# HumanCompatibleAI/overcooked_ai

Hardware: NVIDIA H100
Metric: env-steps/sec (joint transitions) (higher is better)
Workload: dtype int32

## Files before the change

### overcooked_ai_b200/csrc/ovc_b200.cu

```cuda
#include <cuda.h>
#include <cuda_runtime.h>
#include <stdint.h>
#include <stdio.h>
#include <stdlib.h>
#include <string.h>

#include "../../include/ovc_b200.h"
#include "ovc_step.cuh"

namespace ovc {

static thread_local char g_err[512] = "";

static int fail(int code, const char *msg) {
    snprintf(g_err, sizeof g_err, "%s", msg);
    return code;
}
static int fail(int code, const char *msg, long long value) {
    snprintf(g_err, sizeof g_err, "%s (got %lld)", msg, value);
    return code;
}
static int cuda_fail(cudaError_t e, const char *what) {
    snprintf(g_err, sizeof g_err, "%s: %s", what, cudaGetErrorString(e));
    return OVC_E_CUDA;
// ... 225 lines not shown
        else bulk_load_1d(tile, a.state + env0 * S, live_bytes, bar);
    }
    int2 act = make_int2(OVC_A_STAY, OVC_A_STAY);
    if (live) act = load_action<WIDE>(a, env);
    __syncthreads();
    mbar_wait(bar, 0);
    asm volatile("griddepcontrol.launch_dependents;" ::: "memory");

    if (live) {
        SmemRec<S, IO == 1 ? C::SWZ : 0> r{tile, (uint32_t)threadIdx.x * S * 4};
        auto run = [&](auto tb) {
            for (int t = 0; t < T; t++) {
                const long long idx = (long long)t * a.n_envs + env;
                int2 nxt = act;
                if (t + 1 < T) nxt = load_action<WIDE>(a, idx + a.n_envs);
                StepOut o;
                step_core<RS>(r, tb, a.start_records, S, act.x, act.y, a.horizon, a.flags, RS ? &a.rs : nullptr, env, a.n_layouts, o);
                write_outputs<WIDE>(a, idx, o);
                act = nxt;
            }
        };
        if (n_tbl) run(TblS{tbl});
        else run(TblG{reinterpret_cast<const char *>(a.layouts)});
    }
    fence_async_smem();
    __syncthreads();
    if (threadIdx.x == 0) {
        if (IO == 1) tma_store_2d(&tmap, 0, (int)(env0 * C::ROWS_PER_ENV), tile);
        else bulk_store_1d(a.state + env0 * S, tile, live_bytes);
        bulk_commit();
        bulk_wait_read<0>();
    }
}

}

#include "ovc_rollout.cuh"

namespace ovc {

__global__ void reset_kernel(const int32_t *__restrict__ start_records, int n_layouts, int32_t *__restrict__ state,
                             const int32_t *__restrict__ env_layout, const int32_t *__restrict__ mask,
                             long long n_envs, int S) {
    const int cpr = S / 4;
    const long long i = (long long)blockIdx.x * blockDim.x + threadIdx.x;
    if (i >= n_envs * cpr) return;
    const long long env = i / cpr;
    const int c = (int)(i % cpr);
    if (mask && mask[env] == 0) return;
    int lid = env_layout ? env_layout[env] : (state[env * S + 3] & 0xFF);
    if (lid < 0 || lid >= n_layouts) lid = 0;
    reinterpret_cast<int4 *>(state)[i] = __ldg(reinterpret_cast<const int4 *>(start_records) + (long long)lid * cpr + c);
}

__global__ void reset_random_kernel(const ovc_layout_t *__restrict__ layouts, int n_layouts,
                                    const int32_t *__restrict__ start_records, int32_t *__restrict__ state,
                                    const int32_t *__restrict__ env_layout, const int32_t *__restrict__ mask,
                                    long long n_envs, int S, const ovc_random_start_t rs) {
    const long long env = (long long)blockIdx.x * blockDim.x + threadIdx.x;
    if (env >= n_envs) return;
    if (mask && mask[env] == 0) return;
    int32_t *rec = state + env * S;
    const unsigned old = (unsigned)rec[3];
    int lid = env_layout ? env_layout[env] : (int)(old & 0xFF);
    const unsigned episode = ((old >> 16) + 1u) & 0xFFFFu;
    if (rs.random_layout) lid = random_layout_id(rs, (uint64_t)env, episode, n_layouts);
    if (lid < 0 || lid >= n_layouts) lid = 0;
    const ovc_layout_t *L = layouts + lid;
    random_start_record([&](int w, int32_t v) { rec[w] = v; }, S, start_records + (size_t)lid * S, L->cook_time, L->free_pos,
                        L->n_free, L->n_pots, lid, rs, (uint64_t)env, episode);
}

typedef CUresult (*encode_tiled_fn)(CUtensorMap *, CUtensorMapDataType, cuuint32_t, void *, const cuuint64_t *,
                                    const cuuint64_t *, const cuuint32_t *, const cuuint32_t *, CUtensorMapInterleave,
                                    CUtensorMapSwizzle, CUtensorMapL2promotion, CUtensorMapFloatOOBfill);

static encode_tiled_fn get_encode_fn() {
    static encode_tiled_fn fn = nullptr;
    static bool tried = false;
    if (!tried) {
        tried = true;
        void *p = nullptr;
        cudaDriverEntryPointQueryResult q;
        if (cudaGetDriverEntryPoint("cuTensorMapEncodeTiled", &p, cudaEnableDefault, &q) == cudaSuccess &&
            q == cudaDriverEntryPointSuccess)
            fn = (encode_tiled_fn)p;
    }
    return fn;
}

template <int S>
static int make_tmap(CUtensorMap *m, int32_t *state, long long n_envs, int box_rows = Cfg<S>::BOX_ROWS) {
    using C = Cfg<S>;
    encode_tiled_fn enc = get_encode_fn();
    if (!enc) return fail(OVC_E_CUDA, "cuTensorMapEncodeTiled entry point not available");
    cuuint64_t dims[2] = {(cuuint64_t)C::ROW_WORDS, (cuuint64_t)(n_envs * C::ROWS_PER_ENV)};
    cuuint64_t strides[1] = {(cuuint64_t)C::ROW_WORDS * 4};
    cuuint32_t box[2] = {(cuuint32_t)C::ROW_WORDS, (cuuint32_t)box_rows};
    cuuint32_t estr[2] = {1, 1};
    CUresult r = enc(m, CU_TENSOR_MAP_DATA_TYPE_INT32, 2, state, dims, strides, box, estr, CU_TENSOR_MAP_INTERLEAVE_NONE,
                     S == 16 ? CU_TENSOR_MAP_SWIZZLE_64B : CU_TENSOR_MAP_SWIZZLE_128B, CU_TENSOR_MAP_L2_PROMOTION_NONE,
                     CU_TENSOR_MAP_FLOAT_OOB_FILL_NONE);
    if (r != CUDA_SUCCESS) return fail(OVC_E_CUDA, "cuTensorMapEncodeTiled failed", (long long)r);
    return OVC_OK;
}

struct OutFmt {
    int act, sparse, shaped, done, events;
    bool stream;
    bool missing(const void *act_p, const void *sparse_p, const void *shaped_p, const void *done_p, const void *events_p) const {
        return !act_p || !events_p || (sparse && !sparse_p) || (shaped && !shaped_p) || (done && !stream && !done_p);
    }
    bool wide() const { return act == 8 && sparse == 4; }
};

static OutFmt formats_of(int flags) {
    OutFmt f;
    f.act = (flags & OVC_F_ACT_PACKED) ? 1 : (flags & OVC_F_ACT_U8) ? 2 : 8;
    f.stream = flags & OVC_F_OUT_STREAM;
    if (f.stream) f.sparse = 2, f.shaped = 0, f.done = 2, f.events = 4;
    else if (flags & OVC_F_OUT_CODES) f.sparse = 0, f.shaped = 0, f.done = 0, f.events = 2;
    else if (flags & OVC_F_OUT_PACKED) f.sparse = 2, f.shaped = 2, f.done = 0, f.events = 2;
    else if (flags & OVC_F_OUT_NARROW) f.sparse = 2, f.shaped = 2, f.done = 1, f.events = 8;
    else f.sparse = 4, f.shaped = 8, f.done = 4, f.events = 8;
    return f;
}

template <int S, int IO>
static cudaError_t launch_one(const CUtensorMap &tmap, const StepArgs &a, unsigned grid, size_t smem, cudaStream_t st) {
    using C = Cfg<S>;
    cudaLaunchConfig_t cfg;
    memset(&cfg, 0, sizeof cfg);
    cfg.gridDim = dim3(grid), cfg.blockDim = dim3(C::TILE), cfg.dynamicSmemBytes = smem, cfg.stream = st;
    cudaLaunchAttribute attr[1];
    attr[0].id = cudaLaunchAttributeProgrammaticStreamSerialization;
    attr[0].val.programmaticStreamSerializationAllowed = 1;
    cfg.attrs = attr;
    cfg.numAttrs = (a.flags & OVC_F_PDL) ? 1 : 0;
    const bool wide = formats_of(a.flags).wide();
    if (a.has_rs)
        return wide ? cudaLaunchKernelEx(&cfg, step_kernel<S, IO, true, true>, tmap, a)
                    : cudaLaunchKernelEx(&cfg, step_kernel<S, IO, true, false>, tmap, a);
    return wide ? cudaLaunchKernelEx(&cfg, step_kernel<S, IO, false, true>, tmap, a)
                : cudaLaunchKernelEx(&cfg, step_kernel<S, IO, false, false>, tmap, a);
}

template <int S, int TILE>
static int launch_rollout(const StepArgs &a, cudaStream_t st) {
    using C = RollCfg<S, TILE>;
    CUtensorMap tmap;
    memset(&tmap, 0, sizeof tmap);
    int rc = make_tmap<S>(&tmap, a.state, a.n_envs, C::BOX_ROWS);
    if (rc) return rc;
    const size_t smem = C::smem_bytes(a.n_layouts);
    const OutFmt f = formats_of(a.flags);
    const bool wide = f.wide(), stream = f.stream;
    void (*kern)(const CUtensorMap, const StepArgs) =
        a.has_rs ? (wide ? rollout_kernel<S, TILE, true, FMT_WIDE> : stream ? rollout_kernel<S, TILE, true, FMT_STREAM> : rollout_kernel<S, TILE, true, FMT_HOST>)
                 : (wide ? rollout_kernel<S, TILE, false, FMT_WIDE> : stream ? rollout_kernel<S, TILE, false, FMT_STREAM> : rollout_kernel<S, TILE, false, FMT_HOST>);
    if (smem > 48 * 1024) {
        cudaError_t e = cudaFuncSetAttribute(kern, cudaFuncAttributeMaxDynamicSharedMemorySize, (int)smem);
        if (e != cudaSuccess) return cuda_fail(e, "rollout kernel shared-memory attribute");
    }
    const long long grid = (a.n_envs + TILE - 1) / TILE;
    StepArgs ka = a;
    ka.flags &= ~F_K5_NO_PREFETCH;
#if OVC_K5_PREFETCH > 1
    {
        int dev = 0, n_sm = 0, per_sm = 0;
        cudaError_t e = cudaGetDevice(&dev);
        if (e == cudaSuccess) e = cudaDeviceGetAttribute(&n_sm, cudaDevAttrMultiProcessorCount, dev);
        if (e == cudaSuccess) e = cudaOccupancyMaxActiveBlocksPerMultiprocessor(&per_sm, kern, TILE, smem);
        if (e != cudaSuccess) return cuda_fail(e, "rollout kernel occupancy");
        const long long warps = grid * (TILE / 32);
        if (grid <= (long long)per_sm * n_sm && (warps >= 24LL * n_sm || warps < 12LL * n_sm)) ka.flags |= F_K5_NO_PREFETCH;
    }
#endif
    cudaLaunchConfig_t cfg;
    memset(&cfg, 0, sizeof cfg);
    cfg.gridDim = dim3((unsigned)grid), cfg.blockDim = dim3(TILE), cfg.dynamicSmemBytes = smem, cfg.stream = st;
    cudaLaunchAttribute attr[1];
    attr[0].id = cudaLaunchAttributeProgrammaticStreamSerialization;
    attr[0].val.programmaticStreamSerializationAllowed = 1;
    cfg.attrs = attr;
    cfg.numAttrs = 0;
    cudaError_t e = cudaLaunchKernelEx(&cfg, kern, tmap, ka);
    if (e != cudaSuccess) return cuda_fail(e, "rollout kernel launch");
    return OVC_OK;
}

static int rollout_tile(int S, long long n_envs, int n_layouts) {
    static int forced = -1;
    if (forced < 0) {
        const char *e = getenv("OVC_K5_TILE");
        forced = e ? atoi(e) : 0;
    }
    (void)n_envs;
    if (S > 32) return 64;
    if (forced == 32 || forced == 64 || forced == 128) return forced;
    return n_layouts >= 3 ? 128 : 64;
}

static bool use_rollout_kernel(const StepArgs &a, int io) {
    static int off = -1;
    if (off < 0) {
        const char *e = getenv("OVC_K5_LEGACY");
        off = e && atoi(e) ? 1 : 0;
    }
    const bool stream = a.flags & OVC_F_OUT_STREAM;
    return (!off || stream) && (a.n_steps > 1 || stream) && a.n_steps <= ROLLOUT_MAX_STEPS && io == 1 && a.n_layouts <= MAX_SMEM_LAYOUTS;
}

template <int S>
static int launch_rollout_tiled(const StepArgs &a, cudaStream_t st) {
    if constexpr (S > 32) {
        return launch_rollout<S, 64>(a, st);
    } else {
        switch (rollout_tile(S, a.n_envs, a.n_layouts)) {
        case 32: return launch_rollout<S, 32>(a, st);
        case 64: return launch_rollout<S, 64>(a, st);
        default: return launch_rollout<S, 128>(a, st);
        }
    }
}

template <int S>
static int launch_rollout_any(const StepArgs &a0, cudaStream_t st) {
    long long max_steps = 0xFFFFFFFFLL / a0.n_envs - 1;
    {
        static long long cap = -1;
        if (cap < 0) {
            const char *e = getenv("OVC_K5_MAX_LAUNCH_STEPS");
            cap = e ? atoll(e) : 0;
        }
        if (cap > 0 && cap < max_steps && !(a0.flags & OVC_F_OUT_STREAM)) max_steps = cap;
    }
    if (a0.n_steps <= max_steps) return launch_rollout_tiled<S>(a0, st);
    if (max_steps < 1 || (a0.flags & OVC_F_OUT_STREAM)) return fail(OVC_E_UNSUPPORTED, "rollout too large for one launch (n_steps * n_envs must stay below 2^32)");
    const OutFmt f = formats_of(a0.flags);
    for (long long t0 = 0; t0 < a0.n_steps; t0 += max_steps) {
        StepArgs a = a0;
        const long long off = t0 * a0.n_envs;
        a.n_steps = (int)(a0.n_steps - t0 < max_steps ? a0.n_steps - t0 : max_steps);
        a.actions = reinterpret_cast<const int32_t *>(reinterpret_cast<const char *>(a0.actions) + off * f.act);
        if (a0.sparse) a.sparse = reinterpret_cast<int32_t *>(reinterpret_cast<char *>(a0.sparse) + off * f.sparse);
        if (a0.shaped) a.shaped = reinterpret_cast<int32_t *>(reinterpret_cast<char *>(a0.shaped) + off * f.shaped);
        if (a0.done) a.done = reinterpret_cast<int32_t *>(reinterpret_cast<char *>(a0.done) + off * f.done);
        a.events = reinterpret_cast<int32_t *>(reinterpret_cast<char *>(a0.events) + off * f.events);
        const int rc = launch_rollout_tiled<S>(a, st);
        if (rc) return rc;
    }
    return OVC_OK;
}

template <int S>
static int launch_step(const StepArgs &a, int io, cudaStream_t st) {
    using C = Cfg<S>;
    if (use_rollout_kernel(a, io)) return launch_rollout_any<S>(a, st);
    const unsigned grid = (unsigned)((a.n_envs + C::TILE - 1) / C::TILE);
    CUtensorMap tmap;
    memset(&tmap, 0, sizeof tmap);
    const int n_tbl = a.n_layouts <= MAX_SMEM_LAYOUTS ? a.n_layouts : 0;
    const size_t smem = io == 3 ? 0 : C::TILE_BYTES + (size_t)n_tbl * sizeof(ovc_layout_t) + 16;
    cudaError_t e;
    if (io == 1) {
        int rc = make_tmap<S>(&tmap, a.state, a.n_envs);
        if (rc) return rc;
        e = launch_one<S, 1>(tmap, a, grid, smem, st);
    } else if (io == 2) {
        e = launch_one<S, 2>(tmap, a, grid, smem, st);
    } else {
        e = launch_one<S, 3>(tmap, a, grid, smem, st);
    }
    if (e != cudaSuccess) return cuda_fail(e, "step kernel launch");
    return OVC_OK;
}

static int check_common(const void *layouts, int n_layouts, const void *state, long long n_envs, int S) {
    if (!layouts || !state) return fail(OVC_E_BADARG, "null pointer argument");
    if (n_layouts <= 0 || n_layouts > 256) return fail(OVC_E_BADARG, "n_layouts must be 1..256", (long long)(n_layouts));
    if (n_envs < 0) return fail(OVC_E_BADARG, "negative n_envs");
    if (S != 16 && S != 32 && S != 64 && S != 128)
        return fail(OVC_E_BADARG, "state_words must be 16, 32, 64 or 128", (long long)(S));
    if (((uintptr_t)state & 15) != 0) return fail(OVC_E_BADARG, "state must be 16-byte aligned");
    return OVC_OK;
}

static int step_impl(const void *layouts, int n_layouts, const int32_t *start_records, int32_t *state,
                     const int32_t *actions, int32_t *sparse, int32_t *shaped, int32_t *done, int32_t *events,
                     long long n_envs, int n_steps, int S, int horizon, int flags, const ovc_random_start_t *rs,
                     void *stream) {
    int rc = check_common(layouts, n_layouts, state, n_envs, S);
    if (rc) return rc;
    const OutFmt f = formats_of(flags);
    if (f.stream && (flags & (OVC_F_OUT_CODES | OVC_F_OUT_PACKED | OVC_F_OUT_NARROW)))
        return fail(OVC_E_BADARG, "OVC_F_OUT_STREAM excludes the other output formats");
    if (!start_records || f.missing(actions, sparse, shaped, done, events)) return fail(OVC_E_BADARG, "null pointer argument");
    if (!f.sparse) sparse = nullptr;
    if (!f.shaped) shaped = nullptr;
    if (!f.done) done = nullptr;
    if (f.stream && (((unsigned)flags >> OVC_F_STREAM_CAP_SHIFT) & 0xFFFFu) == 0)
        return fail(OVC_E_BADARG, "OVC_F_OUT_STREAM needs a capacity in flags bits 16-31");
    auto misaligned = [](const void *p, int bytes) { return bytes > 1 && (uintptr_t)p % (uintptr_t)bytes != 0; };
    if (misaligned(actions, f.act) || misaligned(sparse, f.sparse) || misaligned(shaped, f.shaped) || misaligned(done, f.done) ||
        misaligned(events, f.events))
        return fail(OVC_E_BADARG, "actions / sparse / shaped / done / events must be aligned to their element size");
    if (n_steps < 1) return fail(OVC_E_BADARG, "n_steps must be >= 1");
    if (n_envs == 0) return OVC_OK;
    int io = (flags & OVC_F_IO_MASK) >> OVC_F_IO_SHIFT;
    if (io == 0) io = 1;
    if (io < 1 || io > 3) return fail(OVC_E_BADARG, "unknown record I/O strategy", (long long)(io));
    if (io == 1 && (n_envs * (S / (S == 16 ? 16 : 32))) > 0x7FFFFFFFLL) io = 2;
    if (f.stream && (io != 1 || n_layouts > MAX_SMEM_LAYOUTS || n_steps > ROLLOUT_MAX_STEPS))
        return fail(OVC_E_UNSUPPORTED, "OVC_F_OUT_STREAM needs the rollout kernel: default record I/O, at most 8 layouts");
    StepArgs a{(const ovc_layout_t *)layouts, start_records, state, actions, sparse, shaped, done, events,
               n_envs, n_layouts, n_steps, horizon, flags, rs != nullptr, rs ? *rs : ovc_random_start_t{0, 0, 0}};
    cudaStream_t st = (cudaStream_t)stream;
    switch (S) {
    case 16: return launch_step<16>(a, io, st);
    case 32: return launch_step<32>(a, io, st);
    case 64: return launch_step<64>(a, io, st);
    default: return launch_step<128>(a, io, st);
    }
}

}
// ... 452 lines not shown
```

### overcooked_ai_b200/csrc/ovc_rollout.cuh

```cuda
#pragma once

#ifndef OVC_K5_PREFETCH
#define OVC_K5_PREFETCH 4
#endif

namespace ovc {

struct Derived {
    uint16_t face[1024];
    uint8_t move[2048];
    int32_t cook5[32];
    int32_t deliver5[32];
    uint8_t potcode5[32][2];
    uint8_t dcode5[32];
    uint8_t pad[32];
};
static_assert(sizeof(Derived) == 4480, "Derived table size");
constexpr int DERIVED_ZERO_CHUNKS = (1024 * 2 + 2048) / 16;
#define OVC_DOFF(field) ((uint32_t)offsetof(Derived, field))
#define OVC_LOFF(field) ((uint32_t)offsetof(ovc_layout_t, field))

constexpr unsigned POT_FROZEN = 1u << 31;
constexpr int ROLLOUT_MAX_STEPS = 1 << 22;

// ... 40 lines not shown
        return (1u << b) | ((unsigned)((c - 1) & 1) << (b + 1));
    }
    if (c == 7) return 1u << OVC_EV_SOUP_PICKUP;
    if (c <= 13) {
        const int b = (0x0C0207 >> (((c - 8) >> 1) * 8)) & 0xFF;
        return (1u << b) | ((unsigned)((c - 8) & 1) << (b + 1));
    }
    if (c == 14) return 1u << OVC_EV_SOUP_DROP;
    if (c <= 22) {
        const int tom = (c - 15) >> 2, cls = (c - 15) & 3;
        const unsigned base = 1u << (tom ? OVC_EV_POTTING_TOMATO : OVC_EV_POTTING_ONION);
        const unsigned opt = 1u << (OVC_EV_OPTIMAL_ONION_POTTING + tom), via = 1u << (OVC_EV_VIABLE_ONION_POTTING + tom);
        const unsigned cat = 1u << (OVC_EV_CATASTROPHIC_ONION_POTTING + tom), usl = 1u << (OVC_EV_USELESS_ONION_POTTING + tom);
        return base | (cls == 0 ? (opt | via) : cls == 1 ? via : cls == 2 ? cat : (opt | usl));
    }
    return (1u << OVC_EV_SOUP_DELIVERY) | (delivery_row((unsigned)(c - 23)) << OVC_EV_RECIPE_SHIFT);
}

template <int S, int SWZ>
struct TileRec {
    uint32_t rec;
    uint32_t xm;
    __device__ __forceinline__ TileRec(uint32_t tile, int tid) {
        rec = tile + (uint32_t)tid * S * 4;
        if (SWZ == 0) xm = 0;
        else if (S <= 32) xm = ((((uint32_t)tid * S * 4) >> 7) & ((1u << SWZ) - 1u)) << 4;
        else xm = (uint32_t)tid * (S / 32);
    }
    __device__ __forceinline__ uint32_t phys(uint32_t off) const {
        if (SWZ == 0) return off;
        if (S <= 32) return off ^ xm;
        return off ^ (((xm + (off >> 7)) & 7u) << 4);
    }
    __device__ __forceinline__ int4 ld4(int c) const { return lds_tile4(rec + phys((uint32_t)c * 16)); }
    __device__ __forceinline__ void st4(int c, int4 v) const { sts_tile4(rec + phys((uint32_t)c * 16), v); }
    __device__ __forceinline__ uint32_t addr(int w) const { return rec + phys((uint32_t)w * 4); }
    __device__ __forceinline__ unsigned ldw(int w) const { return lds_tile(addr(w)); }
    __device__ __forceinline__ void stw(int w, unsigned v) const { sts_tile(addr(w), v); }
};

__device__ __forceinline__ unsigned pot_to_chip(unsigned w, uint32_t D, unsigned clk) {
    const unsigned tp1 = (w >> 8) & 0x3FFFu;
    if ((w & 7u) != OVC_O_SOUP || tp1 == 0) return w & 0x3FFFFFu;
    const unsigned cook = lds_tbl32(D + OVC_DOFF(cook5) + 4u * ((w >> 3) & 31u));
    if (tp1 - 1u > cook) return (w & 0x3FFFFFu) | POT_FROZEN;
    return (w & 0xFFu) | ((clk + (cook - (tp1 - 1u)) + 1u) << 8);
}
__device__ __forceinline__ unsigned pot_to_ext(unsigned w, uint32_t D, unsigned clk) {
    if (w & POT_FROZEN) return w & 0x3FFFFFu;
    const unsigned g = w >> 8;
    if (g == 0) return w;
    const unsigned cook = lds_tbl32(D + OVC_DOFF(cook5) + 4u * ((w >> 3) & 31u));
    const unsigned left = g - 1u > clk ? g - 1u - clk : 0u;
    return (w & 0xFFu) | ((cook - left + 1u) << 8);
}

struct RollOut {
    int sparse, sh0, sh1;
    unsigned c0, c1;
};

constexpr unsigned PS_FULL = 1u, PS_DISH = 1u << 4;
template <class R>
__device__ __forceinline__ unsigned pot_summary(const R &r, int n_pots) {
    unsigned ps = 0;
#pragma unroll 1
    for (int k = 0; k < n_pots; k++) {
        const unsigned w = r.ldw(4 + k);
        const bool soup = (w & 7u) == OVC_O_SOUP;
        const bool idle = (w >> 8) == 0;
        const unsigned n = (w >> 3) & 3u;
        if (soup && (!idle || n == 3u)) ps += PS_FULL;
        if (soup && (!idle || n == 1u || n == 2u)) ps += PS_DISH;
    }
    return ps;
}

template <class R>
__device__ __forceinline__ unsigned interact_v2(const R &r, uint32_t L, uint32_t D, unsigned &me, const unsigned other_t,
                                                unsigned &misc, const unsigned ps, unsigned &psn, const int n_pots,
                                                const bool old_dyn, const unsigned s, int &sparse, int &shaped) {
    const unsigned cell = lds_tbl16(D + OVC_DOFF(face) + 2u * (me & 0x3FFu));
    const unsigned terr = cell & 7u;
    unsigned held = me >> 10;
    const unsigned ht = held & 7u;
    unsigned code = 0;
    if (terr - 1u < 4u) {
        const bool ctr = terr == OVC_T_COUNTER;
        const uint32_t wa = r.addr(4 + (int)(cell >> 8));
        unsigned cw = terr - 1u;
        if (ctr) cw = lds_tile(wa);
        const bool pick = held == 0 && cw != 0;
        const bool drop = ctr && held != 0 && cw == 0;
        if (pick || drop) {
            const unsigned ot = (held | cw) & 7u;
            const unsigned n_full = ps & 15u;
            bool u;
            if (ot == OVC_O_DISH)
                u = pick ? ((misc & 0xFF00u) == 0 && (other_t == OVC_O_DISH ? 1u : 0u) < (ps >> 4)) : (n_full == 0 && other_t != OVC_O_ONION);
            else
                u = ot <= OVC_O_TOMATO && pick != (n_full == (unsigned)n_pots && other_t != OVC_O_DISH);
            code = 2u * ot + (pick ? 0xFFFFFFFFu : 6u) + (unsigned)u;
            if (ctr) {
                sts_tile(wa, held);
                if (ot == OVC_O_DISH) misc += pick ? 0xFFFFFF00u : 0x100u;
            } else {
                if (ot == OVC_O_TOMATO) code = 0;
                if (ot == OVC_O_DISH && u) shaped += (int)lds_tbl32(L + OVC_LOFF(rew_dish_pickup));
            }
            held = pick ? cw : 0u;
        }
    } else if (terr == OVC_T_POT) {
        const uint32_t wa = r.addr(4 + (int)(cell >> 8));
        const unsigned w = lds_tile(wa);
        const unsigned k5 = (w >> 3) & 31u;
        const unsigned n = k5 & 3u;
        if (ht == 0) {
            if (!old_dyn && (w & ~0xF8u) == OVC_O_SOUP && n != 0) {
                sts_tile(wa, w | ((s + lds_tbl32(D + OVC_DOFF(cook5) + 4u * k5) + 1u) << 8));
                psn += n == 3u ? PS_DISH : PS_FULL;
            }
        } else if (ht == OVC_O_DISH) {
            const unsigned g = w >> 8;
            if ((int)w < 0 || g - 1u <= s) {
                code = 7;
                held = pot_to_ext(w, D, s);
                sts_tile(wa, 0u);
                shaped += (int)lds_tbl32(L + OVC_LOFF(rew_soup_pickup));
                psn -= PS_FULL + PS_DISH;
            }
        } else if (ht <= OVC_O_TOMATO) {
            if ((w >> 8) == 0 && n < 3u) {
                const unsigned tom = ht == OVC_O_TOMATO;
                code = lds_tbl8(D + OVC_DOFF(potcode5) + 2u * k5 + tom);
                sts_tile(wa, ((w ? w : (unsigned)OVC_O_SOUP) + 8u) | (tom << (5 + n)));
                shaped += (int)lds_tbl32(L + OVC_LOFF(rew_placement_in_pot));
                held = 0;
                psn += n == 0 ? PS_DISH : n == 2u ? PS_FULL - PS_DISH : 0u;
            }
        }
    } else if (terr == OVC_T_SERVE && ht == OVC_O_SOUP) {
        const unsigned k5 = (held >> 3) & 31u;
        sparse += (int)lds_tbl32(D + OVC_DOFF(deliver5) + 4u * k5);
        code = lds_tbl8(D + OVC_DOFF(dcode5) + k5);
        held = 0;
    }
    me = (me & 0x3FFu) | (held << 10);
    return code;
}

constexpr int FMT_WIDE = 0, FMT_HOST = 1, FMT_STREAM = 2;

constexpr int F_K5_NO_PREFETCH = 1 << 12;

template <int FMT>
struct RollIO {
    static constexpr bool WIDE = FMT == FMT_WIDE;
    const StepArgs &a;
    unsigned oi, ai;
    const unsigned n;
    unsigned live_mask, cnt, cap, lane_lt, mi, n_groups;
    unsigned short *vals;
    bool leader;
    __device__ __forceinline__ RollIO(const StepArgs &args, long long env, unsigned live) : a(args), n((unsigned)args.n_envs) {
        oi = ai = (unsigned)env;
        live_mask = live, cnt = 0, cap = 0, lane_lt = 0, mi = 0, n_groups = 0, vals = nullptr, leader = false;
        if (FMT == FMT_STREAM) {
            n_groups = (unsigned)((a.n_envs + 31) >> 5);
            mi = (unsigned)(env >> 5);
            cap = ((unsigned)a.flags >> OVC_F_STREAM_CAP_SHIFT) & 0xFFFFu;
            const unsigned lane = (unsigned)env & 31u;
            lane_lt = (1u << lane) - 1u, leader = lane == 0;
            vals = reinterpret_cast<unsigned short *>(a.sparse) + (size_t)mi * cap;
        }
    }
    __device__ __forceinline__ int2 load_action() const { return ovc::load_action<WIDE>(a, ai); }
    __device__ __forceinline__ void next_action() { ai += n; }
    __device__ __forceinline__ void prefetch_action(unsigned rows) const { prefetch_l2(action_addr<WIDE>(a, ai + rows * n)); }
    __device__ __forceinline__ void write(const RollOut &o, int done_v, bool stepped, uint32_t mask) {
        const unsigned i = oi;
        oi += n;
        if (FMT == FMT_STREAM) {
            const unsigned w = o.c0 | (o.c1 << 5) | ((unsigned)done_v << 10) | (stepped ? 1u << 11 : 0u) |
                               (o.sh0 != 0 ? 1u << 12 : 0u) | (o.sh1 != 0 ? 1u << 13 : 0u);
            const unsigned m = __ballot_sync(live_mask, w != 0);
            if (leader) reinterpret_cast<unsigned *>(a.events)[mi] = m;
            mi += n_groups;
            if (w != 0) {
                const unsigned pos = cnt + __popc(m & lane_lt);
                if (pos < cap) vals[pos] = (unsigned short)w;
            }
            cnt += __popc(m);
            if (a.done) reinterpret_cast<unsigned short *>(a.done)[i] = (unsigned short)w;
            return;
        }
        if (!WIDE && (a.flags & (OVC_F_OUT_CODES | OVC_F_OUT_PACKED))) {
            unsigned w = o.c0 | (o.c1 << 5) | ((unsigned)done_v << 10) | (stepped ? 1u << 11 : 0u);
            if (a.flags & OVC_F_OUT_CODES) {
                w |= (o.sh0 != 0 ? 1u << 12 : 0u) | (o.sh1 != 0 ? 1u << 13 : 0u);
            } else {
                reinterpret_cast<short *>(a.sparse)[i] = (short)o.sparse;
                reinterpret_cast<char2 *>(a.shaped)[i] = make_char2((signed char)o.sh0, (signed char)o.sh1);
            }
            reinterpret_cast<unsigned short *>(a.events)[i] = (unsigned short)w;
            return;
        }
        const unsigned e0 = stepped ? (unsigned)OVC_EVF_STEPPED_DONE : lds_tbl32(mask + 4u * o.c0);
        const unsigned e1 = stepped ? (unsigned)OVC_EVF_STEPPED_DONE : lds_tbl32(mask + 4u * o.c1);
        if (!WIDE && (a.flags & OVC_F_OUT_NARROW)) {
            reinterpret_cast<short *>(a.sparse)[i] = (short)o.sparse;
            reinterpret_cast<unsigned char *>(a.done)[i] = (unsigned char)done_v;
            reinterpret_cast<char2 *>(a.shaped)[i] = make_char2((signed char)o.sh0, (signed char)o.sh1);
        } else {
            a.sparse[i] = o.sparse;
            a.done[i] = done_v;
            reinterpret_cast<int2 *>(a.shaped)[i] = make_int2(o.sh0, o.sh1);
        }
        reinterpret_cast<int2 *>(a.events)[i] = make_int2((int)e0, (int)e1);
    }
};

template <int S, int TILE>
struct RollCfg {
    static constexpr int ROW_WORDS = S == 16 ? 16 : 32;
    static constexpr int ROWS_PER_ENV = S / ROW_WORDS;
    static constexpr int BOX_ROWS = TILE * ROWS_PER_ENV;
    static constexpr int SWZ = S == 16 ? 2 : 3;
    static constexpr int TILE_BYTES = TILE * S * 4;
    static_assert(BOX_ROWS <= 256, "TMA box rows");
    static_assert(TILE_BYTES % 1024 == 0, "tile must keep the swizzle alignment of what follows");
    static size_t smem_bytes(int n_layouts) { return (size_t)TILE_BYTES + (size_t)n_layouts * (sizeof(ovc_layout_t) + sizeof(Derived)) + 128 + 16; }
};

template <int S, int TILE, bool RS, int FMT>
__global__ void __launch_bounds__(TILE)
rollout_kernel(const __grid_constant__ CUtensorMap tmap, const StepArgs a) {
    using C = RollCfg<S, TILE>;
    constexpr bool WIDE = FMT == FMT_WIDE;
    const int tid = threadIdx.x;
    const long long env0 = (long long)blockIdx.x * TILE;
    const long long env = env0 + tid;
    const bool live = env < a.n_envs;
    const int T = a.n_steps;
    const int n_tbl = a.n_layouts;

    extern __shared__ __align__(1024) char smem[];
    char *tile = smem;
    ovc_layout_t *tbl = reinterpret_cast<ovc_layout_t *>(smem + C::TILE_BYTES);
    Derived *der = reinterpret_cast<Derived *>(smem + C::TILE_BYTES + (size_t)n_tbl * sizeof(ovc_layout_t));
    unsigned *mask = reinterpret_cast<unsigned *>(reinterpret_cast<char *>(der) + (size_t)n_tbl * sizeof(Derived));
    uint64_t *bar = reinterpret_cast<uint64_t *>(mask + 32);
    const uint32_t tbl_bytes = (uint32_t)n_tbl * (uint32_t)sizeof(ovc_layout_t);

    if (tid == 0) {
        mbar_init(bar, 1);
        mbar_expect_tx(bar, (uint32_t)C::TILE_BYTES + tbl_bytes);
        prefetch_tmap(&tmap);
        bulk_load_1d(tbl, a.layouts, tbl_bytes, bar);
    }
    for (int l = 0; l < n_tbl; l++)
        for (int i = tid; i < DERIVED_ZERO_CHUNKS; i += TILE) reinterpret_cast<int4 *>(der + l)[i] = make_int4(0, 0, 0, 0);
    if (tid < 32) mask[tid] = code_mask_of(tid);
    asm volatile("griddepcontrol.wait;" ::: "memory");
    if (tid == 0) tma_load_2d(tile, &tmap, 0, (int)(env0 * C::ROWS_PER_ENV), bar);
    int2 act = make_int2(OVC_A_STAY, OVC_A_STAY);
    if (live) act = load_action<WIDE>(a, env);
#if OVC_K5_PREFETCH > 1
    const bool prefetch = !(a.flags & F_K5_NO_PREFETCH);
    if (live && prefetch)
        for (int k = 1; k < OVC_K5_PREFETCH && k < T; k++) prefetch_l2(action_addr<WIDE>(a, (unsigned)env + (unsigned)k * (unsigned)a.n_envs));
#endif
    __syncthreads();
    mbar_wait(bar, 0);
    asm volatile("griddepcontrol.launch_dependents;" ::: "memory");

    for (int l = 0; l < n_tbl; l++) {
        const ovc_layout_t *L = tbl + l;
        Derived *D = der + l;
        if (tid < 32) {
            const unsigned k5 = tid;
            const int n = k5 & 3, row = recipe_row5(k5);
            D->cook5[k5] = L->cook_time[row];
            D->deliver5[k5] = L->deliver_value[row];
            D->dcode5[k5] = (uint8_t)(23u + delivery_rank((unsigned)row));
            const int old_val = L->best_value[n ? row : 0];
#pragma unroll
            for (int tom = 0; tom < 2; tom++) {
                int cls = 0;
                if (n < 3) {
                    const int new_val = L->best_value[recipe_row5((k5 + 1u) | ((unsigned)tom << (2 + n)))];
                    cls = new_val > 0 ? (old_val == new_val ? 0 : 1) : (old_val > 0 ? 2 : 3);
                }
                D->potcode5[k5][tom] = (uint8_t)(15 + 4 * tom + cls);
            }
        }
        const int n_free = L->n_free;
        for (int i = tid; i < n_free * 12; i += TILE) {
            const int f = i / 12, d = i - f * 12;
            const int pos = L->free_pos[f];
            if (d < 4) {
                D->face[(d << 8) | pos] = L->cell[(pos + dir_delta(d)) & 0xFF];
            } else {
                const int act_i = d - 4;
                int np = pos;
                if (act_i < 4) {
                    const int tp = (pos + dir_delta(act_i)) & 0xFF;
                    if ((L->cell[tp] & 7) == OVC_T_FLOOR) np = tp;
                }
                D->move[(act_i << 8) | pos] = (uint8_t)np;
            }
        }
    }
    __syncthreads();

    const unsigned live_mask = __ballot_sync(0xFFFFFFFFu, live);
    if (live) {
        const TileRec<S, C::SWZ> r(smem_u32(tile), tid);
        const uint32_t tbl_s = smem_u32(tbl), der_s = smem_u32(der), mask_s = smem_u32(mask);
        int t;
        unsigned toff;
        unsigned p0, p1, misc, ps, psn;
        uint32_t L, D;
        int n_pots;
        bool old_dyn;
        auto load_regs = [&](unsigned clk) {
            const int4 h = r.ld4(0);
            t = h.x, p0 = (unsigned)h.y, p1 = (unsigned)h.z, misc = (unsigned)h.w;
            toff = clk - (unsigned)t;
            unsigned lid = misc & 0xFFu;
            if (lid >= (unsigned)n_tbl) lid = 0;
            L = tbl_s + lid * (uint32_t)sizeof(ovc_layout_t), D = der_s + lid * (uint32_t)sizeof(Derived);
            n_pots = (int)lds_tbl32(L + OVC_LOFF(n_pots));
            old_dyn = (lds_tbl32(L + OVC_LOFF(flags)) & OVC_LAYOUT_OLD_DYNAMICS) != 0;
#pragma unroll 1
            for (int k = 0; k < n_pots; k++) r.stw(4 + k, pot_to_chip(r.ldw(4 + k), D, clk));
            ps = psn = pot_summary(r, n_pots);
        };
        load_regs(0u);

        RollIO<FMT> io(a, env, live_mask);

        auto interact = [&](bool second, RollOut &o) {
            unsigned pa = second ? p1 : p0;
            const unsigned pb = second ? p0 : p1;
            int sh = 0;
            const unsigned c = interact_v2(r, L, D, pa, (pb >> 10) & 7u, misc, ps, psn, n_pots, old_dyn, (unsigned)t + toff, o.sparse, sh);
            if (second) p1 = pa, o.sh1 = sh, o.c1 = c;
            else p0 = pa, o.sh0 = sh, o.c0 = c;
        };
        auto finish = [&](int a0, int a1, const RollOut &o, bool stepped) {
            int done = 1;
            if (!stepped) {
                const unsigned o0 = p0 & 0xFFu, o1 = p1 & 0xFFu;
                unsigned n0 = lds_tbl8(D + OVC_DOFF(move) + ((((unsigned)a0 & 7u) << 8) | o0));
                unsigned n1 = lds_tbl8(D + OVC_DOFF(move) + ((((unsigned)a1 & 7u) << 8) | o1));
                const bool collide = n0 == n1 || (n0 == o1 && n1 == o0);
                if (collide) n0 = o0, n1 = o1;
                if ((unsigned)a0 < 4u) p0 = (p0 & ~0x3FFu) | ((unsigned)a0 << 8) | n0;
                if ((unsigned)a1 < 4u) p1 = (p1 & ~0x3FFu) | ((unsigned)a1 << 8) | n1;
                if (old_dyn) {
#pragma unroll 1
                    for (int k = 0; k < n_pots; k++) {
                        const unsigned w = r.ldw(4 + k);
                        if ((w & ~0xE0u) == (OVC_O_SOUP | (3u << 3))) {
                            r.stw(4 + k, w | (((unsigned)t + toff + lds_tbl32(D + OVC_DOFF(cook5) + 4u * ((w >> 3) & 31u)) + 1u) << 8));
                            psn += PS_DISH;
                        }
                    }
                }
                ps = psn;
                done = a.horizon > 0 && t + 1 >= a.horizon;
            }
            io.write(o, done, stepped, mask_s);
            if (stepped) return;
            if (done && (a.flags & OVC_F_AUTO_RESET)) {
                const unsigned lid0 = misc & 0xFFu;
                if (RS && a.has_rs) {
                    const unsigned episode = ((misc >> 16) + 1u) & 0xFFFFu;
                    int lid = (int)lid0;
                    if (a.rs.random_layout) lid = random_layout_id(a.rs, (uint64_t)env, episode, a.n_layouts);
                    const ovc_layout_t *Ln = tbl + lid;
                    random_start_record([&](int w, int32_t v) { r.stw(w, (unsigned)v); }, S, a.start_records + (size_t)lid * S,
                                        Ln->cook_time, Ln->free_pos, Ln->n_free, Ln->n_pots, lid, a.rs, (uint64_t)env, episode);
                } else {
                    const int4 *__restrict__ src = reinterpret_cast<const int4 *>(a.start_records + (size_t)lid0 * S);
#pragma unroll 4
                    for (int c = 0; c < S / 4; c++) r.st4(c, __ldg(src + c));
                }
                load_regs((unsigned)t + toff + 1u);
            } else {
                t = t + 1;
            }
        };

        for (int s = 0; s < T; s++) {
            int2 nxt = act;
            io.next_action();
            if (s + 1 < T) nxt = io.load_action();
#if OVC_K5_PREFETCH > 1
            if (prefetch && s + OVC_K5_PREFETCH < T) io.prefetch_action(OVC_K5_PREFETCH - 1);
#endif
            const int a0 = act.x, a1 = act.y;
            act = nxt;
            RollOut o{0, 0, 0, 0u, 0u};
            bool stepped = a.horizon > 0 && t >= a.horizon;
            if (FMT != FMT_STREAM) {
                if (stepped) {
                    io.write(o, 1, true, mask_s);
                    continue;
                }
                stepped = false;
            }
            if (!stepped) {
                const bool i0 = a0 == OVC_A_INTERACT, i1 = a1 == OVC_A_INTERACT;
                if (i0 || i1) interact(!i0, o);
                if (i0 && i1) interact(true, o);
            }
            finish(a0, a1, o, FMT == FMT_STREAM && stepped);
        }
#pragma unroll 1
        for (int k = 0; k < n_pots; k++) r.stw(4 + k, pot_to_ext(r.ldw(4 + k), D, (unsigned)t + toff));
        r.st4(0, make_int4(t, (int)p0, (int)p1, (int)misc));
    }
    fence_async_smem();
    __syncthreads();
    if (tid == 0) {
        tma_store_2d(&tmap, 0, (int)(env0 * C::ROWS_PER_ENV), tile);
        bulk_commit();
        bulk_wait_read<0>();
    }
}

}
```

Baseline: 77.41 billion.

## Stage wide rollout outputs in shared memory and flush via bulk async copies

In the wide output format, per-step outputs (sparse reward, done, shaped, events) are written into a double-buffered shared-memory stage holding four steps instead of being stored to global memory directly. Every four steps thread 0 issues cp.async.bulk stores for each row. This replaces scattered per-thread global stores with large contiguous bulk transfers, and the host enables it only when alignment allows and occupancy does not drop below what the grid needs. The cost is extra shared memory and two block-wide barriers per flush, which could stall warps that have diverged in progress.

```diff
diff --git a/overcooked_ai_b200/csrc/ovc_b200.cu b/overcooked_ai_b200/csrc/ovc_b200.cu
--- a/overcooked_ai_b200/csrc/ovc_b200.cu
+++ b/overcooked_ai_b200/csrc/ovc_b200.cu
@@ -401,7 +401,7 @@
     memset(&tmap, 0, sizeof tmap);
     int rc = make_tmap<S>(&tmap, a.state, a.n_envs, C::BOX_ROWS);
     if (rc) return rc;
-    const size_t smem = C::smem_bytes(a.n_layouts);
+    size_t smem = C::smem_bytes(a.n_layouts);
     const OutFmt f = formats_of(a.flags);
     const bool wide = f.wide(), stream = f.stream;
     void (*kern)(const CUtensorMap, const StepArgs) =
@@ -413,14 +413,27 @@
     }
     const long long grid = (a.n_envs + TILE - 1) / TILE;
     StepArgs ka = a;
-    ka.flags &= ~F_K5_NO_PREFETCH;
-#if OVC_K5_PREFETCH > 1
+    ka.flags &= ~(F_K5_NO_PREFETCH | F_K5_STAGE);
+    int dev = 0, n_sm = 0, per_sm = 0;
     {
-        int dev = 0, n_sm = 0, per_sm = 0;
         cudaError_t e = cudaGetDevice(&dev);
         if (e == cudaSuccess) e = cudaDeviceGetAttribute(&n_sm, cudaDevAttrMultiProcessorCount, dev);
         if (e == cudaSuccess) e = cudaOccupancyMaxActiveBlocksPerMultiprocessor(&per_sm, kern, TILE, smem);
         if (e != cudaSuccess) return cuda_fail(e, "rollout kernel occupancy");
+    }
+    if (wide && a.n_envs % 4 == 0 &&
+        !((reinterpret_cast<uintptr_t>(a.sparse) | reinterpret_cast<uintptr_t>(a.done) | reinterpret_cast<uintptr_t>(a.shaped) |
+           reinterpret_cast<uintptr_t>(a.events)) & 15)) {
+        const size_t staged = C::stage_offset(a.n_layouts) + k5_stage_bytes<TILE>();
+        int per_sm_staged = 0;
+        cudaError_t e = staged > 48 * 1024 ? cudaFuncSetAttribute(kern, cudaFuncAttributeMaxDynamicSharedMemorySize, (int)staged) : cudaSuccess;
+        if (e == cudaSuccess) e = cudaOccupancyMaxActiveBlocksPerMultiprocessor(&per_sm_staged, kern, TILE, staged);
+        if (e != cudaSuccess) return cuda_fail(e, "rollout kernel staged occupancy");
+        const long long waves1 = (grid + n_sm - 1) / n_sm, need = waves1 < per_sm ? waves1 : per_sm;
+        if (per_sm_staged >= need) ka.flags |= F_K5_STAGE, smem = staged;
+    }
+#if OVC_K5_PREFETCH > 1
+    {
         const long long warps = grid * (TILE / 32);
         if (grid <= (long long)per_sm * n_sm && (warps >= 24LL * n_sm || warps < 12LL * n_sm)) ka.flags |= F_K5_NO_PREFETCH;
     }
diff --git a/overcooked_ai_b200/csrc/ovc_rollout.cuh b/overcooked_ai_b200/csrc/ovc_rollout.cuh
--- a/overcooked_ai_b200/csrc/ovc_rollout.cuh
+++ b/overcooked_ai_b200/csrc/ovc_rollout.cuh
@@ -216,13 +216,24 @@
 constexpr int FMT_WIDE = 0, FMT_HOST = 1, FMT_STREAM = 2;
 
 constexpr int F_K5_NO_PREFETCH = 1 << 12;
-
-template <int FMT>
+constexpr int F_K5_STAGE = 1 << 13;
+
+constexpr int K5_STAGE_R = 4;
+constexpr int K5_STAGE_ROW = 24;
+template <int TILE>
+constexpr size_t k5_stage_bytes() { return 2 * (size_t)K5_STAGE_R * TILE * K5_STAGE_ROW; }
+__device__ __forceinline__ void bulk_store_1d_s(void *dst, uint32_t src, uint32_t bytes) {
+    asm volatile("cp.async.bulk.global.shared::cta.bulk_group [%0], [%1], %2;" ::"l"((uint64_t)dst), "r"(src), "r"(bytes) : "memory");
+}
+
+template <int FMT, int TILE>
 struct RollIO {
     static constexpr bool WIDE = FMT == FMT_WIDE;
     const StepArgs &a;
     unsigned oi, ai;
     const unsigned n;
+    uint32_t stage = 0;
+    unsigned tid = 0, st_r = 0, st_half = 0, st_oi = 0;
     unsigned live_mask, cnt, cap, lane_lt, mi, n_groups;
     unsigned short *vals;
     bool leader;
@@ -237,6 +248,9 @@
             lane_lt = (1u << lane) - 1u, leader = lane == 0;
             vals = reinterpret_cast<unsigned short *>(a.sparse) + (size_t)mi * cap;
         }
+    }
+    __device__ __forceinline__ void stage_outputs(uint32_t base, int thread, long long env0) {
+        stage = base, tid = (unsigned)thread, st_oi = (unsigned)env0;
     }
     __device__ __forceinline__ int2 load_action() const { return ovc::load_action<WIDE>(a, ai); }
     __device__ __forceinline__ void next_action() { ai += n; }
@@ -271,6 +285,15 @@
         }
         const unsigned e0 = stepped ? (unsigned)OVC_EVF_STEPPED_DONE : lds_tbl32(mask + 4u * o.c0);
         const unsigned e1 = stepped ? (unsigned)OVC_EVF_STEPPED_DONE : lds_tbl32(mask + 4u * o.c1);
+        if (WIDE && stage) {
+            const uint32_t row = stage + (st_half * K5_STAGE_R + st_r) * (uint32_t)(TILE * K5_STAGE_ROW);
+            sts_tile(row + tid * 4u, (unsigned)o.sparse);
+            sts_tile(row + TILE * 4 + tid * 4u, (unsigned)done_v);
+            asm volatile("st.shared.v2.u32 [%0], {%1, %2};" ::"r"(row + TILE * 8 + tid * 8u), "r"(o.sh0), "r"(o.sh1) : "memory");
+            asm volatile("st.shared.v2.u32 [%0], {%1, %2};" ::"r"(row + TILE * 16 + tid * 8u), "r"(e0), "r"(e1) : "memory");
+            st_r++;
+            return;
+        }
         if (!WIDE && (a.flags & OVC_F_OUT_NARROW)) {
             reinterpret_cast<short *>(a.sparse)[i] = (short)o.sparse;
             reinterpret_cast<unsigned char *>(a.done)[i] = (unsigned char)done_v;
@@ -281,6 +304,25 @@
             reinterpret_cast<int2 *>(a.shaped)[i] = make_int2(o.sh0, o.sh1);
         }
         reinterpret_cast<int2 *>(a.events)[i] = make_int2((int)e0, (int)e1);
+    }
+    __device__ __forceinline__ void flush_stage() {
+        fence_async_smem();
+        __syncthreads();
+        if (tid == 0) {
+            const uint32_t half = stage + st_half * K5_STAGE_R * (uint32_t)(TILE * K5_STAGE_ROW);
+            for (unsigned q = 0; q < st_r; q++) {
+                const uint32_t row = half + q * (uint32_t)(TILE * K5_STAGE_ROW);
+                const unsigned e = st_oi + q * n;
+                bulk_store_1d_s(a.sparse + e, row, TILE * 4);
+                bulk_store_1d_s(a.done + e, row + TILE * 4, TILE * 4);
+                bulk_store_1d_s(a.shaped + 2 * (size_t)e, row + TILE * 8, TILE * 8);
+                bulk_store_1d_s(a.events + 2 * (size_t)e, row + TILE * 16, TILE * 8);
+            }
+            bulk_commit();
+            bulk_wait_read<1>();
+        }
+        __syncthreads();
+        st_oi += st_r * n, st_r = 0, st_half ^= 1u;
     }
 };
 
@@ -293,7 +335,8 @@
     static constexpr int TILE_BYTES = TILE * S * 4;
     static_assert(BOX_ROWS <= 256, "TMA box rows");
     static_assert(TILE_BYTES % 1024 == 0, "tile must keep the swizzle alignment of what follows");
-    static size_t smem_bytes(int n_layouts) { return (size_t)TILE_BYTES + (size_t)n_layouts * (sizeof(ovc_layout_t) + sizeof(Derived)) + 128 + 16; }
+    __host__ __device__ static size_t smem_bytes(int n_layouts) { return (size_t)TILE_BYTES + (size_t)n_layouts * (sizeof(ovc_layout_t) + sizeof(Derived)) + 128 + 16; }
+    __host__ __device__ static size_t stage_offset(int n_layouts) { return (smem_bytes(n_layouts) + 127) & ~(size_t)127; }
 };
 
 template <int S, int TILE, bool RS, int FMT>
@@ -402,7 +445,8 @@
         };
         load_regs(0u);
 
-        RollIO<FMT> io(a, env, live_mask);
+        RollIO<FMT, TILE> io(a, env, live_mask);
+        if (WIDE && (a.flags & F_K5_STAGE) && env0 + TILE <= a.n_envs) io.stage_outputs(smem_u32(smem + C::stage_offset(n_tbl)), tid, env0);
 
         auto interact = [&](bool second, RollOut &o) {
             unsigned pa = second ? p1 : p0;
@@ -458,6 +502,7 @@
         };
 
         for (int s = 0; s < T; s++) {
+            if (WIDE && io.stage && io.st_r == K5_STAGE_R) io.flush_stage();
             int2 nxt = act;
             io.next_action();
             if (s + 1 < T) nxt = io.load_action();
@@ -482,6 +527,7 @@
             }
             finish(a0, a1, o, FMT == FMT_STREAM && stepped);
         }
+        if (WIDE && io.stage) io.flush_stage();
 #pragma unroll 1
         for (int k = 0; k < n_pots; k++) r.stw(4 + k, pot_to_ext(r.ldw(4 + k), D, (unsigned)t + toff));
         r.st4(0, make_int4(t, (int)p0, (int)p1, (int)misc));
```

New measurement: 56.96 billion (median of 6 runs). -26.4%, worse.
